# jovoy/SolarAxionRayTracing

Hardware: AMD Instinct MI355X
Metric: rays/sec (higher is better)
Workload: dtype f64

## Files before the change

### solaraxionraytracing_amd/csrc/sart_kernels.hip

```cpp
#include <hip/hip_runtime.h>
#include <stdint.h>
#include <string.h>

#include <type_traits>

#include "../../include/sart.h"
#include "sart_device.h"
#include "sart_math.h"

namespace sart {

struct U4 { uint32_t x, y, z, w; };
constexpr int kPhiloxRounds = 7;

__device__ __forceinline__ U4 philox4x32(uint32_t c0, uint32_t c1, uint32_t c2, uint32_t c3, uint32_t k0,
                                         uint32_t k1) {
#pragma unroll
  for (int r = 0; r < kPhiloxRounds; ++r) {
    const uint64_t p0 = (uint64_t)0xD2511F53u * c0;
    const uint64_t p1 = (uint64_t)0xCD9E8D57u * c2;
    const uint32_t hi0 = (uint32_t)(p0 >> 32), lo0 = (uint32_t)p0;
    const uint32_t hi1 = (uint32_t)(p1 >> 32), lo1 = (uint32_t)p1;
    const uint32_t n0 = __builtin_amdgcn_bitop3_b32(hi1, c1, k0, 0x96);
    const uint32_t n2 = __builtin_amdgcn_bitop3_b32(hi0, c3, k1, 0x96);
// ... 349 lines not shown
template <bool WORD = false>
__device__ __forceinline__ void energy_draw_begin(const HotB& HB, int r_idx, double u5, uint32_t word, EnergyDraw& d, int r_idx_guide = -1) {
  if (r_idx_guide < 0) r_idx_guide = r_idx;
  d.u = u5;
  if (WORD) {
    d.khi = word;
  } else {
    const double w = fmin(u5 + 1.0, 1.9999999999999998);
    d.khi = __builtin_amdgcn_alignbit((uint32_t)__double2hiint(w), (uint32_t)__double2loint(w), 20u);
  }
  static_assert((kEnergyGuideDiv & (kEnergyGuideDiv - 1)) == 0 && kEnergyGuideDiv >= 32, "the word form shifts by log2 of it");
  const double v = 1.0 - u5;
  const uint32_t ku = WORD ? word >> (32 - __builtin_ctz((uint32_t)kEnergyGuideDiv)) : (uint32_t)(int)(u5 * (double)kEnergyGuideDiv);
  const uint32_t code = (uint32_t)__double2hiint(v) >> 14;
  const uint32_t kl = (uint32_t)kEnergyGuideUniform + min(kEnergyGuideCode0 - code, (uint32_t)kEnergyGuideLogMax);
  const bool uniform_bucket = WORD ? word < 0xF8000000u : v > 0.03125;
  const uint32_t k = uniform_bucket ? ku : kl;
  d.row = __umul24((uint32_t)r_idx, (uint32_t)HB.cdf_stride);
  d.gword = gload<uint32_t>(HB.energy_guide, (__umul24((uint32_t)r_idx_guide, (uint32_t)kEnergyGuideEntries) + k) * 2u);
}
__device__ __forceinline__ void energy_draw_candidates(const HotB& HB, EnergyDraw& d) {
  d.lo = d.gword & 0xFFFFu;
  d.hi = d.gword >> 16;
  d.c = gload<u4v>(HB.cdf_hi32, (d.row + d.lo) * 4u);
}
template <bool WORD = false>
__device__ __forceinline__ int energy_draw_finish(const HotB& HB, const EnergyDraw& d) {
  const double u = d.u;
  if (WORD) {
    const uint32_t z = d.khi;
    uint32_t lo = d.lo + (uint32_t)(d.c.x < z) + (uint32_t)(d.c.y < z) + (uint32_t)(d.c.z < z) + (uint32_t)(d.c.w < z);
    if ((d.c.w < z) & (d.hi > d.lo + 4u)) {
      asm volatile("; rare: energy bucket wider than four entries");
      uint32_t hi = d.hi;
      while (lo < hi) {
        const uint32_t mid = (lo + hi) >> 1;
        if (gload<double>(HB.diff_flux_cdfs, (d.row + mid) * 8u) < u) lo = mid + 1; else hi = mid;
      }
    }
    return (int)min(lo, (uint32_t)(HB.n_energies - 1));
  }
  const uint32_t km1 = max(d.khi, 1u) - 1u;
  uint32_t lo = d.lo + (uint32_t)(d.c.x < km1) + (uint32_t)(d.c.y < km1) + (uint32_t)(d.c.z < km1) + (uint32_t)(d.c.w < km1);
  const bool tie = ((d.c.x - km1) < 2u) | ((d.c.y - km1) < 2u) | ((d.c.z - km1) < 2u) | ((d.c.w - km1) < 2u);
  if (((d.c.w < km1) & (d.hi > d.lo + 4u)) | tie) {
    asm volatile("; rare: energy bucket wider than four entries, or a tie in the upper 32 bits");
    if (tie) lo = d.lo;
    uint32_t hi = d.hi;
    while (lo < hi) {
      const uint32_t mid = (lo + hi) >> 1;
      if (gload<double>(HB.diff_flux_cdfs, (d.row + mid) * 8u) < u) lo = mid + 1; else hi = mid;
    }
  }
  return (int)min(lo, (uint32_t)(HB.n_energies - 1));
}
template <bool WORD = false>
__device__ __forceinline__ int sample_energy_index(const HotB& HB, int r_idx, double u5, uint32_t word = 0u) {
  EnergyDraw d;
  energy_draw_begin<WORD>(HB, r_idx, u5, word, d);
  energy_draw_candidates(HB, d);
  return energy_draw_finish<WORD>(HB, d);
}

static_assert(sizeof(EnergyDev) == 8 * sizeof(double), "EnergyDev is loaded as eight f64");
__device__ __forceinline__ EnergyDev load_energy_row(const HotB& HB, int e_idx) {
  const uint32_t off = (uint32_t)e_idx * 64u;
  return EnergyDev{gload<double>(HB.energy_tab, off), gload<double>(HB.energy_tab, off + 8u), gload<double>(HB.energy_tab, off + 16u),
                   gload<double>(HB.energy_tab, off + 24u), gload<double>(HB.energy_tab, off + 32u), gload<double>(HB.energy_tab, off + 40u),
                   gload<double>(HB.energy_tab, off + 48u), gload<double>(HB.energy_tab, off + 56u)};
}

__device__ __forceinline__ double spoke_measure(int n, double c) {
  if (n == 16) {
    const double u = HORNER(c, c, -0.5);
    const double v = HORNER(u, u, -0.125);
    const double w = HORNER(v, v, -0.0078125);
    return HORNER(w, w, -1.0 / 32768.0);
  }
  const double t3 = c * HORNER(4.0 * c, c, -3.0);
  return HORNER(2.0 * t3, t3, -1.0);
}

__device__ __forceinline__ void spoke_measure_pair(int n, double ca, double cb, double& ma, double& mb) {
  if (n == 16) {
    const double ua = HORNER(ca, ca, -0.5), ub = HORNER(cb, cb, -0.5);
    const double va = HORNER(ua, ua, -0.125), vb = HORNER(ub, ub, -0.125);
    const double wa = HORNER(va, va, -0.0078125), wb = HORNER(vb, vb, -0.0078125);
    ma = HORNER(wa, wa, -1.0 / 32768.0);
    mb = HORNER(wb, wb, -1.0 / 32768.0);
    return;
  }
  const double ta = ca * HORNER(4.0 * ca, ca, -3.0), tb = cb * HORNER(4.0 * cb, cb, -3.0);
  ma = HORNER(2.0 * ta, ta, -1.0);
  mb = HORNER(2.0 * tb, tb, -1.0);
}

struct Uniforms {
  double u0, u1, u2, u3, u4, u5;
  uint32_t u2_hi;
  uint32_t u5_hi = 0u;
};
__device__ __forceinline__ uint32_t upper32_of_uniform(double u) {
  return (uint32_t)(u * 4294967296.0);
}
struct LaneMasks { uint64_t ok, reached; };

struct BoreRay {
  double x1, y1;
  double x3, y3;
  double sx, sy;
  bool ok;
  uint64_t okm;
};
struct TelRot {
  double rx_c, rx_s, ry_c, ry_s, half_length_telescope;
};
static_assert(offsetof(DevParams, rx_s) == offsetof(DevParams, rx_c) + 8 && offsetof(DevParams, ry_c) == offsetof(DevParams, rx_c) + 16 &&
                  offsetof(DevParams, ry_s) == offsetof(DevParams, rx_c) + 24 && offsetof(DevParams, half_length_telescope) == offsetof(DevParams, rx_c) + 32,
              "TelRot mirrors these five fields of DevParams");
__device__ __forceinline__ const TelRot& tel_rot_of(const DevParams& P) { return *reinterpret_cast<const TelRot*>(&P.rx_c); }

template <bool WORD>
__device__ __forceinline__ int radius_draw(const LdsTables& L, uint32_t u2_hi, double u2) {
  const uint32_t khi = u2_hi;
  const uint32_t kb = khi >> 21, kt = (khi >> 17) - ((kRadiusGuideTopStart >> 17) - (uint32_t)(kRadiusGuide + 1));
  const uint32_t k = khi >= kRadiusGuideTopStart ? kt : kb;
  const int lo0 = (int)L.rguide[k];
  const int hi0 = (int)L.rguide[k + 1];
  auto entry = [&](int i) {
    const uint32_t t = L.rcdf_hi[i];
    return WORD ? t : t + (uint32_t)(t != 0xFFFFFFFFu);
  };
  const uint32_t c0 = entry(lo0), c1 = entry(lo0 + 1), c2 = entry(lo0 + 2), c3 = entry(lo0 + 3);
  int lo = lo0 + (int)(c0 < khi) + (int)(c1 < khi) + (int)(c2 < khi) + (int)(c3 < khi);
  bool tie = WORD ? false : min(min(c0 - khi, c1 - khi), min(c2 - khi, c3 - khi)) < 2u;
  if ((c3 < khi) & (hi0 > lo0 + 4)) {
    asm volatile("; rare: radius bucket wider than four entries");
    int hi = hi0;
    while (lo < hi) {
      const int mid = (lo + hi) >> 1;
      if (entry(mid) < khi) lo = mid + 1; else hi = mid;
    }
    if (!WORD) tie = (entry(lo) - khi) < 2u;
  }
  if (!WORD && tie) {
    asm volatile("; rare: a tie in the upper 32 bits of the radius draw");
    lo = lower_bound_bracket(as_global(L.rcdf_f64), lo0, hi0, u2);
  }
  return lo;
}

template <bool FAST, bool ZEXT, bool NOWALL = false, bool WORD = false>
__device__ __forceinline__ void phase_a_bore(const HotA& H, const DevParams& P, const LdsTables& L, const Uniforms& U, RayState& st,
                                             bool& sampled, bool& reached, BoreRay& br, LaneMasks& M) {
  const bool cfg_test = FAST ? false : (H.test_active != 0);
  const double u0 = U.u0, u1 = U.u1, u2 = U.u2, u3 = U.u3, u4 = U.u4;
  st.u5 = U.u5;
  st.u5_hi = U.u5_hi;
  st.r_idx = 0;

  bool ok = true;
  double ex, ey;
  double sx, sy;
  if (!cfg_test) {
    double s1, c1, s2, c2;
    const SinCosCoef K = sincos_coef();
    sincos_turns<2>(u0, L.sincos, K, &s1, &c1);
    sincos_turns<1>(u1, L.sincos, K, &s2, &c2);
    st.r_idx = radius_draw<WORD>(L, U.u2_hi, u2);
    const double r = (0.0015 + (double)st.r_idx * 0.0005) * H.sun_radius;
    const double ox = c1 * s2 * r, oy = s1 * s2 * r, oz = c2 * r - H.sun_distance;
    double sp, cp;
    sincos_turns<2>(u4, L.sincos, K, &sp, &cp);
    const double rr = H.radius_cb * fsqrt_pos(u3 + 1e-300);
    ex = cp * rr;
    ey = sp * rr;
    const double inv_dz = frcp(H.length_b - oz);
    sx = (ex - ox) * inv_dz;
    sy = (ey - oy) * inv_dz;
  } else {
    double sp, cp;
    const SinCosCoef K = sincos_coef();
    sincos_turns<2>(u1, L.sincos, K, &sp, &cp);
    const double rr = P.test_radius * fsqrt(u0);
    const double ox = cp * rr + P.test_x, oy = sp * rr + P.test_y, oz = P.test_z;
    if (P.test_parallel) {
      ex = ox + (u2 * 0.5) - 0.25;
      ey = oy + (u3 * 0.5) - 0.25;
    } else {
      double sq, cq;
      sincos_turns<2>(u3, L.sincos, K, &sq, &cq);
      const double r2 = H.radius_cb * fsqrt(u2);
      ex = cq * r2;
      ey = sq * r2;
    }
    const double inv_dz = frcp(H.length_b - oz);
    sx = (ex - ox) * inv_dz;
    sy = (ey - oy) * inv_dz;
    const double dzc = P.test_collimator_z - H.length_b;
    const double cx = fma(dzc, sx, ex) - P.test_x, cy = fma(dzc, sy, ey) - P.test_y;
    ok = fma(cx, cx, cy * cy) < P.test_radius_sq;
  }
  sampled = ok;
  uint64_t okm = cfg_test ? ballot64(ok) : ~0ull;

  const double A2 = fma(sx, sx, sy * sy);
  const double norm = ZEXT ? 1.0 : fsqrt_pos(1.0 + A2);
  double path_cb = H.length_b * norm;
  bool hits_entrance = true;
  if (!NOWALL) {
    const double x0 = fma(-H.length_b, sx, ex), y0 = fma(-H.length_b, sy, ey);
    hits_entrance = fma(x0, x0, y0 * y0) < H.radius_cb_sq;
  }
  if (!NOWALL && (ok & !hits_entrance)) {
    const double Dm = fma(ex, sx, ey * sy);
    const double c = fma(ex, ex, ey * ey) - H.radius_cb_sq;
    const double sq = fsqrt(fma(Dm, Dm, -A2 * c));
    const double q = (Dm >= 0.0) ? (-Dm - sq) : (-Dm + sq);
    const double qa = q * frcp(A2), cq = c * frcp(q);
    const double t_lo = (Dm >= 0.0) ? qa : cq, t_hi = (Dm >= 0.0) ? cq : qa;
    const double z_hi = H.length_b + t_hi, z_lo = H.length_b + t_lo;
    const bool v1 = (z_hi > 0.0) && (z_hi < H.length_coldbore);
    const bool v2 = (z_lo > 0.0) && (z_lo < H.length_coldbore);
    const double t = v1 ? t_hi : t_lo;
    ok = (v1 != v2);
    path_cb = fabs(t) * norm;
  }
  if (!NOWALL) okm = ballot64(ok);
  st.path_cb = path_cb;
  const double x1 = fma(H.dz1, sx, ex), y1 = fma(H.dz1, sy, ey);
  const double x2 = fma(H.dz2, sx, ex), y2 = fma(H.dz2, sy, ey);
  const double x3 = fma(H.dz3, sx, ex), y3 = fma(H.dz3, sy, ey);
  const bool in1 = fma(x1, x1, y1 * y1) < H.radius_cb_sq, in2 = fma(x2, x2, y2 * y2) < H.pipe1_radius_sq,
             in3 = fma(x3, x3, y3 * y3) < H.pipe1_radius_sq;
  ok = ok & in1 & in2 & in3;
  okm &= ballot64(in1) & ballot64(in2) & ballot64(in3);
  reached = ok;
  M.reached = okm;
  br.x1 = x1; br.y1 = y1; br.x3 = x3; br.y3 = y3; br.sx = sx; br.sy = sy;
  br.ok = ok;
  br.okm = okm;
}

template <bool FAST, int ROT>
__device__ __forceinline__ bool phase_a_telescope(const HotA& H, const DevParams& P, const TelRot& R, const LdsTables& L, const BoreRay& br,
                                                  RayState& st, double& radial_out, LaneMasks& M) {
  const bool cfg_rotated = (ROT < 0) ? (H.rotated != 0) : (ROT != 0);
  const bool cfg_holes = FAST ? false : (H.telescope_kind == SART_TK_XMM && H.inner_blocks < 0);
  const double x1 = br.x1, y1 = br.y1, x3 = br.x3, y3 = br.y3, sx = br.sx, sy = br.sy;
  bool ok = br.ok;
  uint64_t okm = br.okm;

  const double Lp = H.dz3 - H.dz1;
  double X0, Y0, tsx, tsy, zcb;
  if (!cfg_rotated) {
    X0 = x3 - H.entrance_x;
    Y0 = y3 - H.entrance_y;
    tsx = sx;
    tsy = sy;
    zcb = -Lp;
  } else {
    auto rot = [&](double px, double py, double pz, double& qx, double& qy, double& qz) {
      const double zz = pz - R.half_length_telescope;
      const double ax = fma(px, R.rx_c, zz * R.rx_s);
      const double az = fma(zz, R.rx_c, -px * R.rx_s);
      qx = ax;
      qy = fma(py, R.ry_c, -az * R.ry_s);
      qz = fma(az, R.ry_c, py * R.ry_s) + R.half_length_telescope;
    };
    double ax, ay, az, bx, by, bz;
    rot(x1, y1, -Lp, ax, ay, az);
    rot(x3, y3, 0.0, bx, by, bz);
    ax -= H.entrance_x; ay -= H.entrance_y;
    bx -= H.entrance_x; by -= H.entrance_y;
    const double inv = frcp(bz - az);
    tsx = (bx - ax) * inv;
    tsy = (by - ay) * inv;
    X0 = fma(-az, tsx, ax);
    Y0 = fma(-az, tsy, ay);
    zcb = az;
  }
  st.X0 = X0; st.Y0 = Y0; st.tsx = tsx; st.tsy = tsy; st.zcb = zcb;
  const double Q0 = fma(X0, X0, Y0 * Y0);
  const double inv_radial = frsq(Q0);
  const double radial = Q0 * inv_radial;

  if (H.telescope_kind != SART_TK_LLNL) {
    const bool inner_le = radial <= H.inner_radius, inner_lt = radial < H.inner_radius;
    const bool inner = (H.telescope_kind == SART_TK_XMM) ? inner_le : inner_lt;
    const bool ring_a = radial < H.ring_hi, ring_b = radial > H.ring_lo;
    const bool ring = (H.telescope_kind == SART_TK_XMM) & ring_a & ring_b;
    const double c_ent = X0 * inv_radial;
    const double xs = fma(H.spider_z, tsx, X0), ys = fma(H.spider_z, tsy, Y0);
    const double c_sp = xs * frsq(fma(xs, xs, ys * ys));
    double meas_a, meas_b;
    spoke_measure_pair(H.spoke_n, c_ent, c_sp, meas_a, meas_b);
    const bool spoke_a = meas_a >= H.spoke_cos_thr, spoke_b = meas_b >= H.spoke_cos_thr;
    const bool spoke = spoke_a | spoke_b;
    bool blocked = inner | ring | spoke;
    const bool xmm = H.telescope_kind == SART_TK_XMM;
    uint64_t blocked_m = (xmm ? ballot64(inner_le) : ballot64(inner_lt)) | (xmm ? (ballot64(ring_a) & ballot64(ring_b)) : 0ull) |
                         ballot64(spoke_a) | ballot64(spoke_b);
    if (cfg_holes) {
      const int nH = P.number_of_holes;
      const int lim = nH - (int)ceil((double)nH / 2.0);
      bool res = false, done = false;
      for (int l = -lim; l <= lim; ++l) {
        double hx = 0.0, hy = 0.0;
        if (l != 0) {
          if ((abs(l) & 1) == 0) hy += 2.0 * (double)l * P.hole_in_optics;
          else hx += 2.0 * ((double)l + ((double)l / (double)abs(l))) * P.hole_in_optics;
        }
        const double ix = X0 - hx, iy = Y0 - hy, rad = P.hole_in_optics;
        const double tx = ix / sqrt(2.0) - iy / sqrt(2.0), ty = ix / sqrt(2.0) + iy / sqrt(2.0);
        const double axx = fabs(ix), ayy = fabs(iy), atx = fabs(tx), aty = fabs(ty);
        bool through = false;
        switch (P.hole_type) {
          case SART_HT_CIRCLE: through = sqrt(fma(ix, ix, iy * iy)) < rad; break;
          case SART_HT_CROSS:
            through = (axx < rad && ayy < rad * 16.0) || (ayy < rad && axx < rad * 16.0); break;
          case SART_HT_STAR:
            through = (axx < rad && ayy < rad * 16.0) || (ayy < rad && axx < rad * 16.0) ||
                      (atx < rad && aty < rad * 16.0) || (aty < rad && atx < rad * 16.0); break;
          case SART_HT_SQUARE: through = axx < rad && ayy < rad; break;
          case SART_HT_DIAMOND: through = atx < rad && aty < rad; break;
          default: through = false;
        }
        if (!done) { res = !through; done = through; }
      }
      if (inner) blocked = res;
      blocked_m = ballot64(blocked);
    }
    ok = ok & !blocked;
    okm &= ~blocked_m;
  }

  const bool beyond = radial > H.r1_last;
  ok = ok & !beyond;
  okm &= ~ballot64(beyond);
  const int nS = H.n_shells;
  const int j0 = (int)L.lut[max(min((int)(radial * H.lut_inv_step), H.lut_n - 1), 0)];
  const int jc = min(j0, nS - 1), jb = max(jc - 1, 0);
  const double c_r1 = L.shells[jc].r1, c_ro = L.shells[jc].r1_outer;
  const double b_r1 = L.shells[jb].r1, b_ro = L.shells[jb].r1_outer;
  const bool step = (j0 < nS) & !(c_r1 > radial);
  const int j = j0 + (step ? 1 : 0);
  const bool has_shell = j < nS;
  ok = ok & has_shell;
  okm &= ballot64(has_shell);
  const double g_r1 = step ? c_r1 : b_r1, g_ro = step ? c_ro : b_ro;
  const bool gf_a = j > 0, gf_b = radial > g_r1, gf_c = radial < g_ro;
  ok = ok & !(gf_a & gf_b & gf_c);
  const uint64_t step_m = ballot64(j0 < nS) & ~ballot64(c_r1 > radial);
  const uint64_t in_c = ballot64(radial > c_r1) & ballot64(radial < c_ro), in_b = ballot64(radial > b_r1) & ballot64(radial < b_ro);
  okm &= ~(ballot64(gf_a) & ((step_m & in_c) | (~step_m & in_b)));
  M.ok = okm;
  st.shell = min(j, nS - 1);
  radial_out = radial;
  return ok;
}

template <bool FAST, int ROT, bool ZEXT, bool NOWALL = false, bool WORD = false>
__device__ __forceinline__ bool phase_a_core(const HotA& H, const DevParams& P, const LdsTables& L, const Uniforms& U, RayState& st,
                                             bool& sampled, bool& reached, double& radial_out, LaneMasks& M) {
  static_assert(!ZEXT || (FAST && ROT == 0), "the z-extent form needs the magnet-frame slopes in phase B");
  static_assert(!NOWALL || ZEXT, "the constant-path form is a specialisation of the vacuum, unrotated one");
  BoreRay br;
  phase_a_bore<FAST, ZEXT, NOWALL, WORD>(H, P, L, U, st, sampled, reached, br, M);
  return phase_a_telescope<FAST, ROT>(H, P, tel_rot_of(P), L, br, st, radial_out, M);
}

__device__ __forceinline__ Uniforms uniforms_of(uint32_t seed_lo, uint32_t seed_hi, uint64_t ray_id, uint32_t u3_hi) {
  const uint32_t id_lo = (uint32_t)ray_id, id_hi = (uint32_t)(ray_id >> 32);
  const U4 b0 = philox4x32(id_lo, id_hi, 0u, 0u, seed_lo, seed_hi);
  Uniforms U;
  U.u2 = u52(b0.x, 0u);
  U.u2_hi = b0.x;
  U.u5 = u52(b0.z, 0u);
  U.u5_hi = b0.z;
  U.u0 = u52(b0.y & 0xFFFFF800u, 0u);
  U.u1 = u52(b0.w & 0xFFFFF800u, 0u);
  U.u4 = u52((b0.y << 21) | ((b0.w & 0x7FFu) << 10), 0u);
  U.u3 = u52(u3_hi, 0u);
  return U;
}
template <bool FAST, int ROT, bool ZEXT, bool NOWALL = false, bool WORD = true>
__device__ __forceinline__ bool phase_a(const HotA& H, const DevParams& P, const LdsTables& L, uint32_t seed_lo,
                                        uint32_t seed_hi, uint64_t ray_id, uint32_t u3_hi, RayState& st, bool& sampled,
                                        bool& reached, double& radial, LaneMasks& M) {
  return phase_a_core<FAST, ROT, ZEXT, NOWALL, WORD>(H, P, L, uniforms_of(seed_lo, seed_hi, ray_id, u3_hi), st, sampled, reached, radial, M);
}

__device__ __forceinline__ double zcb_rotated(double mx, double my, double mz, double h, double qx, double qy, double tsx, double tsy, double Lp) {
  const double num = -Lp - h - fma(mx, qx, fma(my, qy, -mz * h));
  return num * frcp(fma(mx, tsx, fma(my, tsy, mz)));
}

struct RayOut {
  uint64_t m_nickel = 0, m_till = 0, m_passed = 0;
  bool passed = false;
#ifdef SART_STAGE_TIMING
  uint64_t tb[6] = {0, 0, 0, 0, 0, 0};
#endif
  double px = 0.0, py = 0.0, rdet = 0.0, weight = 0.0, reflect = 0.0;
  int e_idx = 0;
  GasRay gas = {0.0, 0.0, 0.0, 0.0, 0.0};
};

#ifndef SART_GATHER_LIVE
#define SART_GATHER_LIVE 1
#endif
struct EScanGeo {
  double cos_ya, path_cb, distance_pipe_m, xu1, xu2;
  int ia1, ia2;
  uint64_t m_live;
  uint64_t m_chip;
  uint64_t m_strip;
};
template <bool RECORDS, bool FAST, int GAS, bool ZEXT, bool SCAN = false, bool NODRAW = false, bool ESCAN = false>
__device__ __forceinline__ void phase_b(const DevParams& P, const LdsTables& L, const HotB& HB, const TraceArgs& A,
                                        const RayState& st, int e_idx_in, bool live, RayOut& out, sart_axion_t* rec,
                                        EScanGeo* geo = nullptr) {
#ifdef SART_STAGE_TIMING
#define SART_B_STAMP(k, dep) do { asm volatile("" :: "v"(dep)); out.tb[k] = __builtin_readcyclecounter(); } while (0)
#else
#define SART_B_STAMP(k, dep)
#endif
  SART_B_STAMP(0, st.X0);
  constexpr bool WORD = !RECORDS;
  const bool draw_energy = NODRAW ? false : __builtin_amdgcn_readfirstlane(e_idx_in) < 0;
  EnergyDraw ed = {};
#ifdef SART_DEBUG_KNOBS
  const uint32_t dbg = (uint32_t)__builtin_amdgcn_readfirstlane((int)A.flags);
  if (draw_energy) energy_draw_begin<WORD>(HB, (dbg & 0x02000000u) ? (st.r_idx & 15) : st.r_idx, st.u5, st.u5_hi, ed, (dbg & 0x04000000u) ? (st.r_idx & 15) : st.r_idx);
#else
  if (draw_energy) energy_draw_begin<WORD>(HB, st.r_idx, st.u5, st.u5_hi, ed);
#endif
  const ShellDev& sh = L.shells[st.shell];
  const int wolter = __builtin_amdgcn_readfirstlane(P.telescope_wolter);
  static_assert(!ZEXT || GAS >= 0, "the z-extent form needs the stage at compile time");
  static_assert(!SCAN || !RECORDS, "the mass scan accumulates, it writes no records");
  const int stage_gas = (GAS >= 0) ? GAS : __builtin_amdgcn_readfirstlane(P.stage_gas);
  const int test_active = FAST ? 0 : __builtin_amdgcn_readfirstlane(P.test_active);
  const int n_half_strips = __builtin_amdgcn_readfirstlane(P.n_half_strips);
  const uint32_t flags = (uint32_t)__builtin_amdgcn_readfirstlane((int)A.flags);
  const double X0 = st.X0, Y0 = st.Y0, tsx = st.tsx, tsy = st.tsy, zcb = st.zcb;
  const double Q0 = fma(X0, X0, Y0 * Y0);

  const double D0 = fma(X0, tsx, Y0 * tsy);
  const double A0 = fma(tsx, tsx, tsy * tsy);
  const double L0 = 1.0 + A0;
  double z1;
  uint64_t live_m = ballot64(live), hit1_m, hit2_m;
  const bool hit1 = pick_root(A0 - sh.m1_k, D0 + sh.m1_hb, Q0 - sh.m1_cc, 0.0, sh.m1_zhi, z1, hit1_m);
  if (!hit1) z1 = zcb;
  const double m1x = fma(z1, tsx, X0), m1y = fma(z1, tsy, Y0);
  double n1z = wolter ? sh.n1_r3t : sh.n1_tan * fma(-sh.n1_tan, z1, sh.r1);
  if (live & !hit1)
    n1z = normal_z_general(P, sh, 1, m1x, m1y, z1);
  if (draw_energy) energy_draw_candidates(HB, ed);
  double wx = tsx, wy = tsy, wz = 1.0;
  const double N1 = fma(m1x, m1x, fma(m1y, m1y, n1z * n1z));
  double sin_a1, sin_a2;
  const double sin2_a1 = reflect(wx, wy, wz, L0, m1x, m1y, n1z, N1, sin_a1);

  {
    const double lz = P.l_mirror - z1, num = sh.nickel_num;
    bool nick = sin2_a1 * fma(lz, lz, num * num) > num * num;
    uint64_t nick_m = ballot64(nick);
    if (ballot64(!(lz > 0.0))) {
      if (!(lz > 0.0)) nick = fsqrt(sin2_a1 / (1.0 - sin2_a1)) > num / lz;
      nick_m = ballot64(nick);
    }
    const bool upper = st.shell > 0;
    const bool hit_nickel = live & upper & nick;
    out.m_nickel = live_m & ballot64(upper) & nick_m;
    if (RECORDS && hit_nickel) rec->hitNickel = 1;
    live = live & !hit_nickel & hit1;
    live_m = live_m & ~out.m_nickel & hit1_m;
  }

  SART_B_STAMP(1, wz);
  const double inv_wz = frcp(wz);
  const double s2x = wx * inv_wz, s2y = wy * inv_wz;
  const double X1 = fma(-z1, s2x, m1x), Y1 = fma(-z1, s2y, m1y);
  const double A1 = fma(s2x, s2x, s2y * s2y);
  const double D1 = fma(X1, s2x, Y1 * s2y);
  const double Q1 = fma(X1, X1, Y1 * Y1);
  double z2;
  const bool hit2 = pick_root(A1 - sh.m2_k, D1 + sh.m2_hb, Q1 - sh.m2_cc, sh.m2_zlo, sh.m2_zhi, z2, hit2_m);
  live = live & hit2;
  live_m &= hit2_m;
  if (!hit2) z2 = sh.m2_zlo;
  const double m2x = fma(z2, s2x, X1), m2y = fma(z2, s2y, Y1);
  const double n2z = wolter ? sh.n2_r3t * fma(2.0 * (P.l_mirror - z2), sh.n2_invF, 1.0)
                            : sh.n2_tan * fma(-sh.n2_tan, z2 - sh.m2_zlo, sh.m2_rc);
  const double N2 = fma(m2x, m2x, fma(m2y, m2y, n2z * n2z));
  const double sin2_a2 = reflect(wx, wy, wz, L0, m2x, m2y, n2z, N2, sin_a2);

  SART_B_STAMP(2, wz);
  const bool use_refl = !(flags & SART_CF_IGNORE_REFLECTION);
  int ia1 = 0, ia2 = 0;
  double xu1 = 0.0, xu2 = 0.0;
  if (use_refl) {
    const int na2 = HB.refl_n_angles - 2;
    const double amin = P.refl_angle_min, inv_da = P.refl_inv_dangle, da = P.refl_dangle;
    double asin_a1, asin_a2;
    asin_small_pair(sin_a1, sin2_a1, sin_a2, sin2_a2, asin_a1, asin_a2);
    auto angle_cell = [&](double asin_a, double& xu_out) {
      const double alpha = asin_a * 57.29577951308232;
      const double t = (alpha - amin) * inv_da;
      int i = (int)t;
      i = max(min(i, na2), 0);
      xu_out = (alpha - fma((double)i, da, amin)) * inv_da;
      return i;
    };
    ia1 = angle_cell(asin_a1, xu1);
    ia2 = angle_cell(asin_a2, xu2);
  }

#ifdef SART_DEBUG_KNOBS
  const int e_idx = (dbg & 0x01000000u) ? ((draw_energy ? energy_draw_finish<WORD>(HB, ed) : e_idx_in) & 31) : (draw_energy ? energy_draw_finish<WORD>(HB, ed) : e_idx_in);
#else
  const int e_idx = draw_energy ? energy_draw_finish<WORD>(HB, ed) : e_idx_in;
#endif
  SART_B_STAMP(3, e_idx);
  EnergyDev en = {};
  d2 g1 = {1.0, 1.0}, g2 = {1.0, 1.0};
  const bool gather = (RECORDS || !SART_GATHER_LIVE) ? true : __builtin_amdgcn_inverse_ballot_w64(live_m);
  if (!ESCAN && gather) {
    asm volatile("; hot: gathers of the live lanes");
    en = load_energy_row(HB, e_idx);
    if (use_refl) {
      const uint32_t row = __umul24((uint32_t)(sh.refl_row0 + e_idx), (uint32_t)HB.refl_n_angles);
      g1 = gload<d2>(HB.refl, (row + (uint32_t)ia1) * 8u);
      g2 = gload<d2>(HB.refl, (row + (uint32_t)ia2) * 8u);
    }
  }

  const double pmx = fma(m2x, P.pipe_c, z2 * P.pipe_s) - P.d_cb_xray;
  const double pmz = fma(z2, P.pipe_c, -m2x * P.pipe_s);
  const double vx = fma(wx, P.pipe_c, wz * P.pipe_s);
  const double vz = fma(wz, P.pipe_c, -wx * P.pipe_s);
  const double inv_vz = frcp(vz);
  const double nwin = (sh.dist_det - pmz) * inv_vz;
  double pdx = fma(nwin, vx, pmx), pdy = fma(nwin, wy, m2y), pdz = sh.dist_det;

  const double ya = RECORDS ? -atan_small(tsy) * 57.29577951308232 : 0.0;
  const double cos_ya = RECORDS ? cos_small(ya) : cos_yaw_of_slope(tsy);

  if (RECORDS && live) {
    const double nend = (sh.dist_det_end - pmz) * inv_vz;
    const double ddx = (nend - nwin) * vx, ddy = (nend - nwin) * wy;
    rec->deviationDet = sqrt(fma(ddx, ddx, ddy * ddy));
    rec->pointdataXBefore = X0;
    rec->pointdataYBefore = Y0;
    rec->pixvalsX = floor(X0 / (48.0 / 1400.0)) + 700.0;
    rec->pixvalsY = floor(Y0 / (48.0 / 1400.0)) + 700.0;
  }

  const double distance_pipe_m = (pdz - zcb) * 1e-3;
  if (test_active) {
    const bool through = (sh.r1 - fsqrt(Q0)) > 100.0;
    pdx = through ? fma(sh.dist_det_raw, tsx, X0) : pdx;
    pdy = through ? fma(sh.dist_det_raw, tsy, Y0) : pdy;
    pdz = through ? sh.dist_det_raw : pdz;
  }
  pdx -= P.lateral_shift;
  pdy -= P.transversal_shift;

  const double rdet2 = fma(pdx, pdx, pdy * pdy);
  const bool off_window = rdet2 > P.radius_window_sq, off_x = fabs(pdx) > P.chip_cx, off_y = fabs(pdy) > P.chip_cy;
  const bool on_chip = !((!(flags & SART_CF_IGNORE_DET_WINDOW)) & off_window) & !(off_x | off_y);
  const uint64_t on_chip_m = ~(((flags & SART_CF_IGNORE_DET_WINDOW) ? 0ull : ballot64(off_window)) | ballot64(off_x) | ballot64(off_y));
  const double yt = fabs(fma(pdy, P.theta_c, -pdx * P.theta_s));
  bool in_strip = false;
  for (int i = 0; i < n_half_strips; ++i) in_strip = in_strip | ((yt > P.strip_lo[i]) & (yt < P.strip_hi[i]));
  if constexpr (ESCAN) {
    static_assert(!RECORDS && !SCAN && !FAST, "the energy scan accumulates, and it runs on the generic variants");
    geo->cos_ya = cos_ya;
    geo->path_cb = st.path_cb;
    geo->distance_pipe_m = distance_pipe_m;
    geo->xu1 = xu1; geo->xu2 = xu2;
    geo->ia1 = ia1; geo->ia2 = ia2;
    geo->m_live = live_m;
    geo->m_chip = live_m & on_chip_m;
    geo->m_strip = ballot64(in_strip);
    (void)en; (void)g1; (void)g2; (void)on_chip;
    return;
  }

  const double path_cb = st.path_cb;
  double trans_magnet;
  bool prob_deferred = false;
  {
    double prob = 1.0;
    double absorb = 1.0;
    if (!stage_gas) {
      if (!(flags & SART_CF_IGNORE_CONV_PROB)) prob = ZEXT ? (P.conv_k * L0) * (path_cb * path_cb) : P.conv_k * path_cb * path_cb;
    } else {
      const double path_len = ZEXT ? path_cb * fsqrt_pos(L0) : path_cb;
      const double Lnat = path_len * P.gas_inv_hbarc_m;
      if (!(flags & SART_CF_IGNORE_CONV_PROB)) {
        const double g = en.gamma;
        const double eh = exp_neg(-g * Lnat * 0.5);
        out.gas = GasRay{en.inv_two_e_ev, g * g * 0.25, -2.0 * eh, fma(eh, eh, 1.0), Lnat};
        if (RECORDS) prob = gas_conversion_prob(P.gas_dm2_abs, out.gas, P.gas_term1, L.sincos, GasCos::make());
        else prob_deferred = true;
      }
      absorb = exp_neg(-fma(en.mu_pipe, distance_pipe_m, en.mu_magnet * (path_len * 1e-3)));
    }
    trans_magnet = cos_ya * prob * absorb;
  }
  const double reflectv = fma(xu1, g1.y - g1.x, g1.x) * fma(xu2, g2.y - g2.x, g2.x);
  double weight = reflectv * trans_magnet;
  SART_B_STAMP(4, weight);
  if (RECORDS && live) {
    rec->transmissionMagnet = trans_magnet;
    rec->yawAngles = ya;
    rec->reflect = reflectv;
  }

  const bool has_weight = weight != 0.0;
  const bool till_window = live & has_weight;
  out.m_till = live_m & ballot64(has_weight);
  if (RECORDS && till_window) rec->passedTillWindow = 1;
  live = live & on_chip;
  live_m &= on_chip_m;

  const double trans_window = (n_half_strips > 0) ? (in_strip ? en.t_strongback : en.t_window) : 0.0;
  const uint8_t kind_w = in_strip ? SART_MK_SI : SART_MK_SI3N4;
  if (!(flags & SART_CF_IGNORE_DET_WINDOW)) { asm volatile(""); weight *= trans_window; }
  if (!(flags & SART_CF_IGNORE_GAS_ABS)) { asm volatile(""); weight *= en.a_gas; }
  if (!(flags & SART_CF_XRAY_TEST)) { asm volatile(""); weight *= P.exposure; }
  if (!SCAN && prob_deferred) {
    const double prob = gas_conversion_prob(P.gas_dm2_abs, out.gas, P.gas_term1, L.sincos, GasCos::make());
    weight *= prob;
    out.m_till &= ballot64(prob != 0.0);
  }

  SART_B_STAMP(5, weight);
  const bool final_weight = weight != 0.0;
  out.m_passed = live_m & ballot64(final_weight);
  out.passed = RECORDS ? (live & final_weight) : __builtin_amdgcn_inverse_ballot_w64(out.m_passed);
  out.reflect = reflectv;
  out.e_idx = e_idx;
  out.rdet = fsqrt_pos(rdet2 + 1e-300);
  out.px = -pdx + P.chip_cx;
  out.py = pdy + P.chip_cy;
  out.weight = weight;
  if (RECORDS && live) {
    if (n_half_strips > 0) {
      rec->transProbWindow = trans_window;
      rec->energiesAxWindow = en.energy;
      rec->kindsWindow = kind_w;
    }
    rec->transProbArgon = en.a_gas;
    rec->transProbDetector = en.a_gas;
    rec->energiesAxAll = en.energy;
    rec->kinds = SART_MK_AR;
    rec->energiesAx = en.energy;
    rec->shellNumber = st.shell;
    rec->pointdataR = out.rdet;
    rec->pointdataX = out.px;
    rec->pointdataY = out.py;
    rec->weights = weight;
    rec->weightsAll = weight;
    rec->passed = (weight != 0.0) ? 1 : 0;
  }
}

#ifndef SART_PRIO_A1
#define SART_PRIO_A1 2
#endif
#ifndef SART_PRIO_B
#define SART_PRIO_B 3
#endif
#ifndef SART_PRIO_ACC
#define SART_PRIO_ACC 1
#endif
constexpr int kQueue = 128;

struct __align__(16) TablesLds {
  double sincos[2 * kSinCosEntries];
  uint32_t rcdf_hi[kMaxRadii + 4];
  ShellDev shells[kMaxShells];
  uint16_t rguide[kRadiusGuideEntries + 6];
  uint8_t lut[kShellLutMax];
};

struct __align__(16) WaveRings {
  double X0[kQueue], Y0[kQueue], tsx[kQueue], tsy[kQueue];
  double path[kQueue], u5[kQueue];
  int idx[kQueue];
  uint32_t ray[kQueue];
  uint32_t u3hi[kQueue];
};
struct __align__(16) HistRings {
  double X0[kQueue], Y0[kQueue], tsx[kQueue], tsy[kQueue];
  double path[kQueue];
  uint2 cell[kQueue];
  uint32_t ray[kQueue];
  uint32_t u3hi[kQueue];
};
static_assert(sizeof(WaveRings) - sizeof(HistRings) == kQueue * sizeof(uint32_t) && sizeof(HistRings) % 512 == 0 &&
                  (kTileRingCells / kQueue * (sizeof(WaveRings) - sizeof(HistRings))) / sizeof(double) == kTileExtraCells - kRingExtraCells,
              "what ring 1's packed cell frees is what the histogram kernels' image tile grows by");
template <int WAVES, typename Rings = WaveRings>
struct __align__(16) QueueLds {
  Rings w[WAVES];
};

template <int BLOCK>
__device__ __forceinline__ void stage_tables(TablesLds& S, const DevParams& P, const DevTables& T) {
  for (int i = threadIdx.x; i < 2 * kSinCosEntries; i += BLOCK) S.sincos[i] = as_global(T.sincos_tab)[i];
  for (int i = threadIdx.x; i < P.n_radii + 4; i += BLOCK) {
    const double c = (i < P.n_radii) ? as_global(T.flux_radius_cdf)[i] : 1.0;
    const unsigned long long t = __double2ull_rd(c * 4503599627370496.0) >> 20;
    S.rcdf_hi[i] = t > 0xFFFFFFFFull ? 0xFFFFFFFFu : (uint32_t)t;
  }
  for (int i = threadIdx.x; i < kRadiusGuideEntries; i += BLOCK) S.rguide[i] = as_global(T.radius_guide)[i];
  {
    const auto src = as_global(reinterpret_cast<const uint64_t*>(T.shells));
    uint64_t* dst = reinterpret_cast<uint64_t*>(S.shells);
    const int n = P.n_shells * (int)(sizeof(ShellDev) / 8);
    for (int i = threadIdx.x; i < n; i += BLOCK) dst[i] = src[i];
  }
  for (int i = threadIdx.x; i < P.lut_n; i += BLOCK) S.lut[i] = as_global(T.shell_lut)[i];
  __syncthreads();
}

__device__ __forceinline__ void reload_hot(HotA& dst) {
  typedef const __attribute__((address_space(4))) uint32_t* kernarg_ptr;
  kernarg_ptr p = (kernarg_ptr)__builtin_amdgcn_kernarg_segment_ptr();
  asm volatile("" : "+s"(p));
  uint32_t* d = reinterpret_cast<uint32_t*>(&dst);
#pragma unroll
  for (int k = 0; k < (int)(sizeof(HotA) / 4); ++k) d[k] = p[k];
}

struct ZoneTable {
  int32_t n_zones;
  uint32_t zone_reached;
  uint32_t lo[kMaxZones], hi[kMaxZones];
};
static_assert(sizeof(ZoneTable) == sizeof(HotA) - offsetof(HotA, n_zones), "ZoneTable mirrors the tail of HotA");
static_assert(offsetof(WaveRings, u3hi) == offsetof(WaveRings, ray) + kQueue * sizeof(uint32_t) && offsetof(WaveRings, ray) % 8 == 0 &&
                  offsetof(HistRings, u3hi) == offsetof(HistRings, ray) + kQueue * sizeof(uint32_t) && offsetof(HistRings, ray) % 8 == 0,
              "the image tile uses ray + u3hi of every wave as 128 contiguous doubles");
__device__ __forceinline__ void reload_zones(ZoneTable& dst) {
  typedef const __attribute__((address_space(4))) uint32_t* kernarg_ptr;
  kernarg_ptr p = (kernarg_ptr)__builtin_amdgcn_kernarg_segment_ptr() + offsetof(HotA, n_zones) / 4;
  asm volatile("" : "+s"(p));
  uint32_t* d = reinterpret_cast<uint32_t*>(&dst);
#pragma unroll
  for (int k = 0; k < (int)(sizeof(ZoneTable) / 4); ++k) d[k] = p[k];
}

struct HistKernArgs {
  HotA H;
  const DevBlob* blob;
  TraceArgs A;
  double* acc;
  HotB HB;
  ScanArgs SC;
};
static_assert(offsetof(HistKernArgs, H) == 0 && offsetof(HistKernArgs, blob) == (sizeof(HotA) + 7) / 8 * 8 &&
                  offsetof(HistKernArgs, A) == offsetof(HistKernArgs, blob) + 8 &&
                  offsetof(HistKernArgs, acc) == offsetof(HistKernArgs, A) + sizeof(TraceArgs) &&
                  offsetof(HistKernArgs, HB) == offsetof(HistKernArgs, acc) + 8 &&
                  offsetof(HistKernArgs, SC) == offsetof(HistKernArgs, HB) + sizeof(HotB) && sizeof(HotA) % 4 == 0 &&
                  sizeof(TraceArgs) % 8 == 0 && sizeof(HotB) % 8 == 0,
              "reload_hot / reload_zones / reload_kernarg read the arguments at these offsets");
template <typename T>
__device__ __forceinline__ void reload_kernarg(T& dst, size_t byte_offset) {
  static_assert(sizeof(T) % 4 == 0, "dword granularity");
  typedef const __attribute__((address_space(4))) uint32_t* kernarg_ptr;
  kernarg_ptr p = (kernarg_ptr)__builtin_amdgcn_kernarg_segment_ptr() + byte_offset / 4;
  asm volatile("" : "+s"(p));
  uint32_t* d = reinterpret_cast<uint32_t*>(&dst);
#pragma unroll
  for (int k = 0; k < (int)(sizeof(T) / 4); ++k) d[k] = p[k];
}

template <int BLOCK, bool FAST, bool ROT, int GAS, bool PATHC, bool FIXED, bool SCAN = false>
__global__ __launch_bounds__(BLOCK) void trace_histogram_kernel(HotA H, const DevBlob* __restrict__ blob, TraceArgs A,
                                                                double* __restrict__ acc, HotB HBarg, ScanArgs SCarg) {
  struct LdsLayout {
    TablesLds S;
    double tile_extra[kTileExtraCells];
    DevBlob B;
    TraceArgs Ab;
    QueueLds<BLOCK / 64, HistRings> Q;
  };
  __shared__ LdsLayout lds;
  TablesLds& S = lds.S;
  QueueLds<BLOCK / 64, HistRings>& Q = lds.Q;
  static_assert(!PATHC || (FAST && !ROT && GAS >= 0), "the constant-path form belongs to the unrotated specialisations");
  static_assert(!SCAN || GAS != 0, "a mass scan needs the gas stage");
  static_assert(!SCAN || kScanMaxMasses * 2 * kScanLanes <= (BLOCK / 64) * kQueue, "the scan accumulators live in the image tile's 128 doubles per wave");
  __shared__ uint32_t scan_zero[kScanMaxMasses];
  static_assert((BLOCK / 64) * kQueue == kTileRingCells && kImageTileMax * kImageTileMax <= kTileRingCells + kTileExtraCells &&
                    kImageTileExtraMax * kImageTileExtraMax <= kTileExtraCells && BLOCK / 64 == kTileRingCells / kQueue,
                "the LDS image tile (host: kImageTileMax): 128 doubles per wave of this workgroup's rings + the cells behind the tables");
  static_assert((offsetof(LdsLayout, Q) % 512) == 0, "the rings are addressed with ds_*2st64 offsets (units of 512 bytes for 64-bit columns)");
  auto tile_cell_lo = [&](uint32_t t) -> double* {
    return PATHC ? &Q.w[t >> 7].path[t & 127u] : reinterpret_cast<double*>(&Q.w[t >> 7].ray[0]) + (t & 127u);
  };
  auto tile_cell = [&](uint32_t t) -> double* {
    return t < (uint32_t)kTileRingCells ? tile_cell_lo(t) : &lds.tile_extra[t - (uint32_t)kTileRingCells];
  };
  DevBlob& B = lds.B;
  TraceArgs& Ab = lds.Ab;
  {
    const uint64_t* src = reinterpret_cast<const uint64_t*>(blob);
    uint64_t* dst = reinterpret_cast<uint64_t*>(&B);
    for (int i = threadIdx.x; i < (int)(sizeof(DevBlob) / 8); i += BLOCK) dst[i] = src[i];
    if (threadIdx.x == 0) Ab = A;
    __syncthreads();
  }
  const DevParams& Pb = B.P;
  const DevTables& Tb = B.T;
  {
    uint64_t* q = reinterpret_cast<uint64_t*>(&Q);
    for (int i = threadIdx.x; i < (int)(sizeof(Q) / 8); i += BLOCK) q[i] = 0ull;
    for (int i = threadIdx.x; i < kTileExtraCells; i += BLOCK) lds.tile_extra[i] = 0.0;
    if (SCAN && threadIdx.x < kScanMaxMasses) scan_zero[threadIdx.x] = 0u;
  }
  stage_tables<BLOCK>(S, Pb, Tb);
  const LdsTables L{S.sincos, S.rcdf_hi, Tb.flux_radius_cdf, S.rguide, S.shells, S.lut};

  const int lane = threadIdx.x & 63;
  const int wave = __builtin_amdgcn_readfirstlane((int)(threadIdx.x >> 6));
  const uint64_t waves_total = (uint64_t)gridDim.x * (BLOCK / 64);
  const uint64_t wave_global = (uint64_t)blockIdx.x * (BLOCK / 64) + wave;
  const bool early_reject = (SCAN && !PATHC) ? false : H.n_zones > 0;
  const uint64_t first_chunk = A.ray_id_offset >> 8;
  uint64_t id_base = first_chunk << 8;
  asm volatile("" : "+s"(id_base));
  const uint32_t rel_begin = (uint32_t)(A.ray_id_offset & 255u);
  const uint32_t rel_end = rel_begin + (uint32_t)A.n_rays;
  const uint32_t n_chunks = (rel_end + 255u) >> 8;

  uint32_t n_reached = 0, n_shell = 0, n_nickel = 0, n_till = 0, n_passed = 0;
  uint32_t n_outside = 0;
  using Sum = std::conditional_t<FIXED, long long, double>;
  Sum sum_w = 0, sum_w2 = 0, sum_x = 0, sum_y = 0, sum_r = 0;
  long long sum_wo = 0;
#ifdef SART_STAGE_TIMING
  uint64_t cyc_a0 = 0, cyc_a1 = 0, cyc_b = 0, cyc_bs[6] = {0, 0, 0, 0, 0, 0};
#endif
  uint32_t h0 = 0, t0 = 0;
  uint32_t h1 = 0, t1 = 0;

  auto ring_sync = [] {
    __builtin_amdgcn_fence(__ATOMIC_RELEASE, "wavefront");
    __builtin_amdgcn_wave_barrier();
    __builtin_amdgcn_fence(__ATOMIC_ACQUIRE, "wavefront");
  };
  auto prefix_of = [](uint64_t mask) {
    return __builtin_amdgcn_mbcnt_hi((uint32_t)(mask >> 32), __builtin_amdgcn_mbcnt_lo((uint32_t)mask, 0u));
  };

  auto run_phase_a = [&](uint32_t rel, bool valid, uint32_t u3_hi) {
    SART_STAGE_MARK("A1");
    __builtin_amdgcn_s_setprio(SART_PRIO_A1);
    RayState st;
    bool sampled = false, reached = false;
    double radial;
    HotA Hl;
    reload_hot(Hl);
    constexpr bool ZEXT = FAST && !ROT && GAS >= 0;
    LaneMasks M;
    (void)phase_a<FAST, ROT ? 1 : 0, ZEXT, PATHC>(Hl, Pb, L, A.seed_lo, A.seed_hi, id_base + (uint64_t)rel, u3_hi, st, sampled, reached, radial, M);
    const uint64_t valid_m = ballot64(valid);
    n_reached += (uint32_t)__popcll(valid_m & M.reached);
    const uint64_t selected = valid_m & M.ok;
    n_shell += (uint32_t)__popcll(selected);
#ifdef SART_DEBUG_KNOBS
    const uint64_t mask = (A.flags & 0x10000000u) ? 0ull : (selected & ~ballot64(radial < Pb.shell0_miss_radius));
#else
    const uint64_t mask = selected & ~ballot64(radial < Pb.shell0_miss_radius);
#endif
    const bool alive = __builtin_amdgcn_inverse_ballot_w64(mask);
    const uint32_t cnt = (uint32_t)__popcll(mask);
    if (alive) {
      asm volatile("; hot: ring 1 write");
      const uint32_t slot = (t1 + prefix_of(mask)) % kQueue;
      Q.w[wave].X0[slot] = st.X0; Q.w[wave].Y0[slot] = st.Y0;
      Q.w[wave].tsx[slot] = st.tsx; Q.w[wave].tsy[slot] = st.tsy;
      if (!PATHC) Q.w[wave].path[slot] = st.path_cb;
      Q.w[wave].cell[slot] = make_uint2((uint32_t)(st.r_idx | (st.shell << 16)), st.u5_hi);
    }
    t1 += cnt;
    __builtin_amdgcn_s_setprio(0);
  };

  auto run_phase_b = [&](uint32_t n_valid) {
    SART_STAGE_MARK("B");
    __builtin_amdgcn_s_setprio(SART_PRIO_B);
    RayState st;
    const bool valid = (uint32_t)lane < n_valid;
    const uint32_t slot = (h1 + (uint32_t)lane) % kQueue;
    RayOut out;
    {
      st.X0 = Q.w[wave].X0[slot]; st.Y0 = Q.w[wave].Y0[slot];
      st.tsx = Q.w[wave].tsx[slot]; st.tsy = Q.w[wave].tsy[slot];
      st.path_cb = PATHC ? H.length_b : Q.w[wave].path[slot];
      const uint2 cell = Q.w[wave].cell[slot];
      st.u5 = u52(cell.y, 0u);
      st.u5_hi = cell.y;
      if (!ROT) {
        st.zcb = -(H.dz3 - H.dz1);
      } else {
        st.zcb = zcb_rotated(Pb.rx_s, -Pb.rx_c * Pb.ry_s, Pb.rx_c * Pb.ry_c, Pb.half_length_telescope, st.X0 + Pb.entrance_x,
                             st.Y0 + Pb.entrance_y, st.tsx, st.tsy, H.dz3 - H.dz1);
      }
      const int packed = (int)cell.x;
      st.r_idx = packed & 0xFFFF;
      st.shell = packed >> 16;
      const DevBlob& Bo = lds_opaque(B);
      HotB HB;
      reload_kernarg(HB, offsetof(HistKernArgs, HB));
      asm volatile("" :: "s"(HB.cdf_hi32), "s"(HB.energy_guide), "s"(HB.energy_tab), "s"(HB.refl), "s"(HB.refl_n_angles), "s"(HB.cdf_stride));
      phase_b<false, FAST, GAS, FAST && !ROT && GAS >= 0, SCAN>(Bo.P, L, HB, lds_opaque(Ab), st, (!FAST && H.test_active) ? Pb.n_energies : -1, valid, out, nullptr);
      if constexpr (SCAN) {
        SART_STAGE_MARK("SCAN");
        n_passed += (uint32_t)__popcll(out.m_passed);
        struct { int32_t n_masses, pad; } hdr;
        reload_kernarg(hdr, offsetof(HistKernArgs, SC));
        const uint32_t fl = (uint32_t)__builtin_amdgcn_readfirstlane((int)Ab.flags);
        const bool use_prob = !(fl & SART_CF_IGNORE_CONV_PROB) & ((GAS >= 0) ? (GAS == 1) : (__builtin_amdgcn_readfirstlane(Bo.P.stage_gas) != 0));
        const double term1 = Bo.P.gas_term1;
        const GasCos cos_lead = GasCos::make();
        for (int k = 0; k < hdr.n_masses; ++k) {
          asm volatile("; hot: per-mass loop of the fused scan");
          ScanMass M;
          reload_kernarg(M, offsetof(HistKernArgs, SC) + offsetof(ScanArgs, m) + (size_t)k * sizeof(ScanMass));
          double w = out.weight;
          if (use_prob) w *= gas_conversion_prob(M.dm2_abs, out.gas, term1, L.sincos, cos_lead);
          const uint64_t nz = out.m_passed & ballot64(w != 0.0);
          if (nz != out.m_passed) {
            asm volatile("; rare: a conversion probability of exactly zero");
            if (lane == 0) atomicAdd(&scan_zero[k], (uint32_t)__popcll(out.m_passed & ~nz));
          }
          if (__builtin_amdgcn_inverse_ballot_w64(nz)) {
            const uint32_t t = (uint32_t)k * (2u * kScanLanes) + ((uint32_t)lane & (kScanLanes - 1u));
            if constexpr (FIXED) {
              __hip_atomic_fetch_add(reinterpret_cast<unsigned long long*>(tile_cell_lo(t)), (unsigned long long)to_fixed(w, M.fx_scale_w),
                                     __ATOMIC_RELAXED, __HIP_MEMORY_SCOPE_WORKGROUP);
              __hip_atomic_fetch_add(reinterpret_cast<unsigned long long*>(tile_cell_lo(t + kScanLanes)), (unsigned long long)to_fixed(w * w, M.fx_scale_w2),
                                     __ATOMIC_RELAXED, __HIP_MEMORY_SCOPE_WORKGROUP);
            } else {
              __hip_atomic_fetch_add(tile_cell_lo(t), w, __ATOMIC_RELAXED, __HIP_MEMORY_SCOPE_WORKGROUP);
              __hip_atomic_fetch_add(tile_cell_lo(t + kScanLanes), w * w, __ATOMIC_RELAXED, __HIP_MEMORY_SCOPE_WORKGROUP);
            }
          }
        }
      }
    }
    h1 += n_valid;
    if constexpr (SCAN) {
      n_nickel += (uint32_t)__popcll(out.m_nickel);
      __builtin_amdgcn_s_setprio(0);
      return;
    }
    __builtin_amdgcn_s_setprio(SART_PRIO_ACC);
#ifdef SART_STAGE_TIMING
    for (int k = 0; k < 5; ++k) cyc_bs[k] += out.tb[k + 1] - out.tb[k];
    cyc_bs[5] += out.tb[0];
#endif
    n_nickel += (uint32_t)__popcll(out.m_nickel);
    n_till += (uint32_t)__popcll(out.m_till);
    n_passed += (uint32_t)__popcll(out.m_passed);
    if (out.passed) {
      SART_STAGE_MARK("ACC");
      TraceArgs Al;
      reload_kernarg(Al, offsetof(HistKernArgs, A));
      asm volatile("" :: "s"(Al.replicas), "s"(Al.replica_mask), "s"(Al.replica_stride), "s"(Al.image_nx), "s"(Al.image_ny),
                   "s"(Al.image_x_min), "s"(Al.image_y_min), "s"(Al.image_inv_step_x), "s"(Al.image_inv_step_y), "s"(Al.spectra),
                   "s"(Al.tile_x0), "s"(Al.tile_y0), "s"(Al.tile_n), "s"(Al.tile_base));
      long long w_fx = 0;
      if constexpr (FIXED) {
        w_fx = to_fixed(out.weight, Al.fx_scale_w);
        sum_w += w_fx;
        sum_w2 += to_fixed(out.weight * out.weight, Al.fx_scale_w2);
        sum_x += to_fixed(out.px, kFixedPositionScale);
        sum_y += to_fixed(out.py, kFixedPositionScale);
        sum_r += to_fixed(out.rdet, kFixedPositionScale);
      } else {
        sum_w += out.weight;
        sum_w2 = fma(out.weight, out.weight, sum_w2);
        sum_x += out.px;
        sum_y += out.py;
        sum_r += out.rdet;
      }
      const double fx = (out.px - Al.image_x_min) * Al.image_inv_step_x;
      const double fy = (out.py - Al.image_y_min) * Al.image_inv_step_y;
      const int nx = Al.image_nx, ny = Al.image_ny;
      const uint64_t inside_m = ballot64(fx >= 0.0) & ballot64(fx < (double)nx) & ballot64(fy >= 0.0) & ballot64(fy < (double)ny);
      const bool inside = __builtin_amdgcn_inverse_ballot_w64(inside_m);
      n_outside += inside ? 0u : 1u;
      if constexpr (FIXED) {
        if (out.m_passed & ~inside_m) {
          asm volatile("; rare: passed rays outside the image");
          sum_wo += inside ? 0ll : w_fx;
        }
      }
#ifdef SART_DEBUG_KNOBS
      const uint32_t rep_key = (Al.flags & 0x08000000u) ? blockIdx.x : (uint32_t)wave_global;
      double* const img = Al.replicas + (size_t)(rep_key & Al.replica_mask) * (size_t)Al.replica_stride;
#else
      double* const img = Al.replicas + (size_t)((uint32_t)wave_global & Al.replica_mask) * (size_t)Al.replica_stride;
#endif
#ifdef SART_DEBUG_KNOBS
      if (inside && !(Al.flags & 0x40000000u))
#else
      if (inside)
#endif
      {
        const uint32_t ix = (uint32_t)(int)fx, iy = (uint32_t)(int)fy;
        const uint32_t tn = (uint32_t)Al.tile_n;
        const uint32_t tx = ix - (uint32_t)Al.tile_x0, ty = iy - (uint32_t)Al.tile_y0;
        if ((tx < tn) & (ty < tn)) {
          const uint32_t t = ty * tn + tx + (uint32_t)Al.tile_base;
          if constexpr (FIXED)
            __hip_atomic_fetch_add(reinterpret_cast<unsigned long long*>(tile_cell(t)), (unsigned long long)w_fx, __ATOMIC_RELAXED,
// ... 2597 lines not shown
```

Measured before the change: 97.26 billion.

## Wrap phase B live-lane work in a branch region and keep sincos coefficients in VGPRs

Phase B's post-mirror work now runs inside a lambda that executes only when some lane is live. The ballots that build the till, on-chip and passed masks are moved out of that region and recomputed afterwards from values pinned in VGPRs. Separately, the sincos polynomial coefficients are built once per kernel and pinned in VGPRs through asm constraints, then passed into phase A so they are not rematerialized on every call. Together these target wasted work on waves with no live lanes and repeated constant setup, at the cost of more live registers and some possible occupancy pressure.

Result: faster. 100.0 billion, median of 6 (+2.8%).

```diff
diff --git a/solaraxionraytracing_amd/csrc/sart_kernels.hip b/solaraxionraytracing_amd/csrc/sart_kernels.hip
--- a/solaraxionraytracing_amd/csrc/sart_kernels.hip
+++ b/solaraxionraytracing_amd/csrc/sart_kernels.hip
@@ -525,7 +525,7 @@
 
 template <bool FAST, bool ZEXT, bool NOWALL = false, bool WORD = false>
 __device__ __forceinline__ void phase_a_bore(const HotA& H, const DevParams& P, const LdsTables& L, const Uniforms& U, RayState& st,
-                                             bool& sampled, bool& reached, BoreRay& br, LaneMasks& M) {
+                                             bool& sampled, bool& reached, BoreRay& br, LaneMasks& M, const SinCosCoef* held = nullptr) {
   const bool cfg_test = FAST ? false : (H.test_active != 0);
   const double u0 = U.u0, u1 = U.u1, u2 = U.u2, u3 = U.u3, u4 = U.u4;
   st.u5 = U.u5;
@@ -537,7 +537,7 @@
   double sx, sy;
   if (!cfg_test) {
     double s1, c1, s2, c2;
-    const SinCosCoef K = sincos_coef();
+    const SinCosCoef K = held ? *held : sincos_coef();
     sincos_turns<2>(u0, L.sincos, K, &s1, &c1);
     sincos_turns<1>(u1, L.sincos, K, &s2, &c2);
     st.r_idx = radius_draw<WORD>(L, U.u2_hi, u2);
@@ -735,11 +735,11 @@
 
 template <bool FAST, int ROT, bool ZEXT, bool NOWALL = false, bool WORD = false>
 __device__ __forceinline__ bool phase_a_core(const HotA& H, const DevParams& P, const LdsTables& L, const Uniforms& U, RayState& st,
-                                             bool& sampled, bool& reached, double& radial_out, LaneMasks& M) {
+                                             bool& sampled, bool& reached, double& radial_out, LaneMasks& M, const SinCosCoef* held = nullptr) {
   static_assert(!ZEXT || (FAST && ROT == 0), "the z-extent form needs the magnet-frame slopes in phase B");
   static_assert(!NOWALL || ZEXT, "the constant-path form is a specialisation of the vacuum, unrotated one");
   BoreRay br;
-  phase_a_bore<FAST, ZEXT, NOWALL, WORD>(H, P, L, U, st, sampled, reached, br, M);
+  phase_a_bore<FAST, ZEXT, NOWALL, WORD>(H, P, L, U, st, sampled, reached, br, M, held);
   return phase_a_telescope<FAST, ROT>(H, P, tel_rot_of(P), L, br, st, radial_out, M);
 }
 
@@ -760,8 +760,8 @@
 template <bool FAST, int ROT, bool ZEXT, bool NOWALL = false, bool WORD = true>
 __device__ __forceinline__ bool phase_a(const HotA& H, const DevParams& P, const LdsTables& L, uint32_t seed_lo,
                                         uint32_t seed_hi, uint64_t ray_id, uint32_t u3_hi, RayState& st, bool& sampled,
-                                        bool& reached, double& radial, LaneMasks& M) {
-  return phase_a_core<FAST, ROT, ZEXT, NOWALL, WORD>(H, P, L, uniforms_of(seed_lo, seed_hi, ray_id, u3_hi), st, sampled, reached, radial, M);
+                                        bool& reached, double& radial, LaneMasks& M, const SinCosCoef* held = nullptr) {
+  return phase_a_core<FAST, ROT, ZEXT, NOWALL, WORD>(H, P, L, uniforms_of(seed_lo, seed_hi, ray_id, u3_hi), st, sampled, reached, radial, M, held);
 }
 
 __device__ __forceinline__ double zcb_rotated(double mx, double my, double mz, double h, double qx, double qy, double tsx, double tsy, double Lp) {
@@ -782,6 +782,12 @@
 
 #ifndef SART_GATHER_LIVE
 #define SART_GATHER_LIVE 1
+#endif
+#ifndef SART_B_LIVE_REGION
+#define SART_B_LIVE_REGION 1
+#endif
+#ifndef SART_A_SINCOS_VGPR
+#define SART_A_SINCOS_VGPR 1
 #endif
 struct EScanGeo {
   double cos_ya, path_cb, distance_pipe_m, xu1, xu2;
@@ -898,10 +904,17 @@
   const int e_idx = draw_energy ? energy_draw_finish<WORD>(HB, ed) : e_idx_in;
 #endif
   SART_B_STAMP(3, e_idx);
+  constexpr bool REGION = SART_B_LIVE_REGION && SART_GATHER_LIVE && !RECORDS && !ESCAN;
+  const bool gather = (RECORDS || !SART_GATHER_LIVE) ? true : __builtin_amdgcn_inverse_ballot_w64(live_m);
+  const bool r_prob_deferred = REGION && !SCAN && stage_gas != 0 && !(flags & SART_CF_IGNORE_CONV_PROB);
+  double r_pdx, r_pdy, r_rdet2, r_w_till, r_weight, r_reflect, r_prob;
+  GasRay r_gas;
+  out.e_idx = e_idx;
+  auto behind_the_mirrors = [&]() __attribute__((always_inline)) {
+  if constexpr (REGION) asm volatile("; hot: phase B behind the mirrors, live lanes only");
   EnergyDev en = {};
   d2 g1 = {1.0, 1.0}, g2 = {1.0, 1.0};
-  const bool gather = (RECORDS || !SART_GATHER_LIVE) ? true : __builtin_amdgcn_inverse_ballot_w64(live_m);
-  if (!ESCAN && gather) {
+  if (!ESCAN && (REGION || gather)) {
     asm volatile("; hot: gathers of the live lanes");
     en = load_energy_row(HB, e_idx);
     if (use_refl) {
@@ -945,7 +958,8 @@
   const double rdet2 = fma(pdx, pdx, pdy * pdy);
   const bool off_window = rdet2 > P.radius_window_sq, off_x = fabs(pdx) > P.chip_cx, off_y = fabs(pdy) > P.chip_cy;
   const bool on_chip = !((!(flags & SART_CF_IGNORE_DET_WINDOW)) & off_window) & !(off_x | off_y);
-  const uint64_t on_chip_m = ~(((flags & SART_CF_IGNORE_DET_WINDOW) ? 0ull : ballot64(off_window)) | ballot64(off_x) | ballot64(off_y));
+  const uint64_t on_chip_m = REGION ? 0ull : ~(((flags & SART_CF_IGNORE_DET_WINDOW) ? 0ull : ballot64(off_window)) | ballot64(off_x) | ballot64(off_y));
+  if constexpr (REGION) { r_pdx = pdx; r_pdy = pdy; r_rdet2 = rdet2; }
   const double yt = fabs(fma(pdy, P.theta_c, -pdx * P.theta_s));
   bool in_strip = false;
   for (int i = 0; i < n_half_strips; ++i) in_strip = in_strip | ((yt > P.strip_lo[i]) & (yt < P.strip_hi[i]));
@@ -996,10 +1010,11 @@
 
   const bool has_weight = weight != 0.0;
   const bool till_window = live & has_weight;
-  out.m_till = live_m & ballot64(has_weight);
+  if constexpr (REGION) r_w_till = weight;
+  else out.m_till = live_m & ballot64(has_weight);
   if (RECORDS && till_window) rec->passedTillWindow = 1;
   live = live & on_chip;
-  live_m &= on_chip_m;
+  if constexpr (!REGION) live_m &= on_chip_m;
 
   const double trans_window = (n_half_strips > 0) ? (in_strip ? en.t_strongback : en.t_window) : 0.0;
   const uint8_t kind_w = in_strip ? SART_MK_SI : SART_MK_SI3N4;
@@ -1009,19 +1024,28 @@
   if (!SCAN && prob_deferred) {
     const double prob = gas_conversion_prob(P.gas_dm2_abs, out.gas, P.gas_term1, L.sincos, GasCos::make());
     weight *= prob;
-    out.m_till &= ballot64(prob != 0.0);
+    if constexpr (REGION) r_prob = prob;
+    else out.m_till &= ballot64(prob != 0.0);
   }
 
   SART_B_STAMP(5, weight);
   const bool final_weight = weight != 0.0;
-  out.m_passed = live_m & ballot64(final_weight);
-  out.passed = RECORDS ? (live & final_weight) : __builtin_amdgcn_inverse_ballot_w64(out.m_passed);
-  out.reflect = reflectv;
-  out.e_idx = e_idx;
-  out.rdet = fsqrt_pos(rdet2 + 1e-300);
-  out.px = -pdx + P.chip_cx;
-  out.py = pdy + P.chip_cy;
-  out.weight = weight;
+  if constexpr (!REGION) {
+    out.m_passed = live_m & ballot64(final_weight);
+    out.passed = RECORDS ? (live & final_weight) : __builtin_amdgcn_inverse_ballot_w64(out.m_passed);
+  }
+  if constexpr (REGION) {
+    r_reflect = reflectv; r_weight = weight;
+    if constexpr (SCAN) r_gas = out.gas;
+  } else {
+    out.reflect = reflectv;
+    out.rdet = fsqrt_pos(rdet2 + 1e-300);
+    out.weight = weight;
+  }
+  if constexpr (!REGION) {
+    out.px = -pdx + P.chip_cx;
+    out.py = pdy + P.chip_cy;
+  }
   if (RECORDS && live) {
     if (n_half_strips > 0) {
       rec->transProbWindow = trans_window;
@@ -1040,6 +1064,26 @@
     rec->weights = weight;
     rec->weightsAll = weight;
     rec->passed = (weight != 0.0) ? 1 : 0;
+  }
+  };
+  if constexpr (REGION) {
+    uint32_t flags_j = flags;
+    asm volatile("" : "+s"(flags_j));
+    if (gather) behind_the_mirrors();
+    asm volatile("" : "+v"(r_pdx), "+v"(r_pdy), "+v"(r_rdet2), "+v"(r_w_till), "+v"(r_weight));
+    out.m_till = live_m & ballot64(r_w_till != 0.0);
+    if (r_prob_deferred) out.m_till &= ballot64(r_prob != 0.0);
+    const uint64_t off_m = ((flags_j & SART_CF_IGNORE_DET_WINDOW) ? 0ull : ballot64(r_rdet2 > P.radius_window_sq)) | ballot64(fabs(r_pdx) > P.chip_cx) |
+                           ballot64(fabs(r_pdy) > P.chip_cy);
+    out.m_passed = live_m & ~off_m & ballot64(r_weight != 0.0);
+    out.reflect = r_reflect; out.weight = r_weight;
+    out.rdet = fsqrt_pos(r_rdet2 + 1e-300);
+    if constexpr (SCAN) out.gas = r_gas;
+    out.passed = __builtin_amdgcn_inverse_ballot_w64(out.m_passed);
+    out.px = -r_pdx + P.chip_cx;
+    out.py = r_pdy + P.chip_cy;
+  } else {
+    behind_the_mirrors();
   }
 }
 
@@ -1235,6 +1279,10 @@
     return __builtin_amdgcn_mbcnt_hi((uint32_t)(mask >> 32), __builtin_amdgcn_mbcnt_lo((uint32_t)mask, 0u));
   };
 
+  constexpr bool HOLD_SINCOS = SART_A_SINCOS_VGPR && FAST && GAS == 0 && !SCAN;
+  SinCosCoef Ksc = {-0.5992645293207921, 2.5501640398773455, -5.16771278004997, 3.141592653589793, -1.3352627688545895, 4.0587121264167685,
+                    -4.934802200544679};
+  if constexpr (HOLD_SINCOS) asm volatile("" : "+v"(Ksc.s3), "+v"(Ksc.s2), "+v"(Ksc.s1), "+v"(Ksc.s0), "+v"(Ksc.d3), "+v"(Ksc.d2), "+v"(Ksc.d1));
   auto run_phase_a = [&](uint32_t rel, bool valid, uint32_t u3_hi) {
     SART_STAGE_MARK("A1");
     __builtin_amdgcn_s_setprio(SART_PRIO_A1);
@@ -1245,7 +1293,8 @@
     reload_hot(Hl);
     constexpr bool ZEXT = FAST && !ROT && GAS >= 0;
     LaneMasks M;
-    (void)phase_a<FAST, ROT ? 1 : 0, ZEXT, PATHC>(Hl, Pb, L, A.seed_lo, A.seed_hi, id_base + (uint64_t)rel, u3_hi, st, sampled, reached, radial, M);
+    (void)phase_a<FAST, ROT ? 1 : 0, ZEXT, PATHC>(Hl, Pb, L, A.seed_lo, A.seed_hi, id_base + (uint64_t)rel, u3_hi, st, sampled, reached, radial, M,
+                                                  HOLD_SINCOS ? &Ksc : nullptr);
     const uint64_t valid_m = ballot64(valid);
     n_reached += (uint32_t)__popcll(valid_m & M.reached);
     const uint64_t selected = valid_m & M.ok;
```
